# locuslab/lcp-physics

Hardware: NVIDIA H100
Metric: LCP solves/sec (LCPFunction fwd+bwd, batch=4096 x 64 contacts, fp32) (higher is better)
Workload: dtype f32 I/O and iterates; the condensed n x n KKT matrix is formed, factored and solved in f64

## Files before the change

lcp_physics_b200/csrc/lcp_condensed.cuh:

```cuda
#pragma once
#include "lcp_device.cuh"

namespace lcpb200 {
namespace cnd {

constexpr int NT = 256;
constexpr int UC = 8;
constexpr int CSMAX = 6;
constexpr int KS = 8;
constexpr int LMAX = 16;
constexpr int LU_BW = 2;
constexpr int MISC_BAND_LU = 4;
constexpr int CFLAG_DENSE_LU = 4;
constexpr int STATUS_UNSUPPORTED = -100;

struct CPlan {
  int ok;
  int n, m, e, N, NP, NS;
  int pcap;
  int wcap;
  int smem_bytes;
  int ctas_per_sm;
  int flags;
  int sbytes;
  int o_K, o_W, o_scr, o_bx, o_rdiag, o_Fd, o_Gd, o_As, o_x, o_rx, o_dx, o_qd, o_y, o_ry, o_dy,
      o_s, o_z, o_d, o_rz, o_ds, o_dz, o_rs2, o_red, o_rows, o_posof, o_clist, o_ccols, o_ncols, o_clcnt, o_misc;
};

__host__ __device__ inline size_t al16(size_t x) { return (x + 15) & ~(size_t)15; }
__host__ __device__ inline size_t scratch_bytes(int n, int m, int tsize) {
  return al16((size_t)2 * KS * m * 2) + al16((size_t)2 * KS * m * tsize) + al16((size_t)5 * m * 4) +
         al16((size_t)CSMAX * m * 2) + al16((size_t)8 * m * 4) + al16((size_t)LMAX * n * 2) + al16((size_t)n * 4) + 64;
}

inline size_t carve_plan(CPlan& P, int tsize) {
  size_t o = 0;
  const int n = P.n, m = P.m, e = P.e, NP = P.NP, pcap = P.pcap, wcap = P.wcap;
#define CND_TAKE(field, bytes) do { P.field = (int)o; o += al16((size_t)(bytes)); } while (0)
  size_t kb = (size_t)NP * NP * 8;
  if (scratch_bytes(n, m, tsize) > kb) kb = scratch_bytes(n, m, tsize);
  if ((size_t)8 * NP * 8 > kb) kb = (size_t)8 * NP * 8;
  { const size_t qn = (NP + 31) / 32, sl = (size_t)(NP / qn) * qn * qn * 32 * 8; if (sl > kb) kb = sl; }
  CND_TAKE(o_K, kb);
  CND_TAKE(o_W, (size_t)wcap * 8);
  CND_TAKE(o_scr, (size_t)pcap * 8);
  CND_TAKE(o_bx, (size_t)NP * 8);
  CND_TAKE(o_rdiag, (size_t)NP * 8);
  CND_TAKE(o_Fd, (size_t)wcap * tsize);
  CND_TAKE(o_Gd, (size_t)UC * pcap * tsize);
  CND_TAKE(o_As, (size_t)e * n * tsize);
  CND_TAKE(o_x, n * tsize); CND_TAKE(o_rx, n * tsize); CND_TAKE(o_dx, n * tsize); CND_TAKE(o_qd, n * tsize);
  CND_TAKE(o_y, e * tsize); CND_TAKE(o_ry, e * tsize); CND_TAKE(o_dy, e * tsize);
  CND_TAKE(o_s, m * tsize); CND_TAKE(o_z, m * tsize); CND_TAKE(o_d, m * tsize); CND_TAKE(o_rz, m * tsize);
  CND_TAKE(o_ds, m * tsize); CND_TAKE(o_dz, m * tsize); CND_TAKE(o_rs2, m * tsize);
  CND_TAKE(o_red, 192 * tsize);
  CND_TAKE(o_rows, pcap * 2);
  CND_TAKE(o_posof, m * 2);
  CND_TAKE(o_clist, LMAX * n * 2);
  CND_TAKE(o_ccols, UC * pcap);
  CND_TAKE(o_ncols, pcap);
  CND_TAKE(o_clcnt, n);
  CND_TAKE(o_misc, 16 * 4);
#undef CND_TAKE
  P.sbytes = 16 + (P.o_x - P.o_Fd) + (P.o_y - P.o_qd) + (P.o_misc - P.o_rows);
  return o;
}

extern __shared__ __align__(16) unsigned char cnd_smem[];

template <typename T>
struct CSmem {
  const CPlan& P;
  __device__ __forceinline__ explicit CSmem(const CPlan& p) : P(p) {}
#define CND_ACC(name, type) __device__ __forceinline__ type* name() const { return reinterpret_cast<type*>(cnd_smem + P.o_##name); }
  CND_ACC(K, double) CND_ACC(W, double) CND_ACC(scr, double) CND_ACC(bx, double) CND_ACC(rdiag, double)
  CND_ACC(Fd, T) CND_ACC(Gd, T) CND_ACC(As, T)
  CND_ACC(x, T) CND_ACC(rx, T) CND_ACC(dx, T) CND_ACC(qd, T) CND_ACC(y, T) CND_ACC(ry, T) CND_ACC(dy, T)
  CND_ACC(s, T) CND_ACC(z, T) CND_ACC(d, T) CND_ACC(rz, T) CND_ACC(ds, T) CND_ACC(dz, T) CND_ACC(rs2, T)
  CND_ACC(red, T)
  CND_ACC(rows, unsigned short) CND_ACC(posof, unsigned short) CND_ACC(clist, unsigned short)
  CND_ACC(ccols, unsigned char) CND_ACC(ncols, unsigned char) CND_ACC(clcnt, unsigned char)
  CND_ACC(misc, int)
#undef CND_ACC
};

struct Struct {
  int ncomp, cs;
  int sh;
  int m;
};

enum { CPH_STRUCT = 0, CPH_WINV, CPH_ASSEMBLE, CPH_LU, CPH_SOLVE_RHS, CPH_SOLVE_TRI, CPH_SOLVE_POST, CPH_RESID,
       CPH_STEP, CPH_GRADS, CPH_COUNT };
template <bool ON>
struct Prof {
  long long* p;
  long long t;
  __device__ __forceinline__ explicit Prof(long long* p_) : p(p_), t(0) {}
  __device__ __forceinline__ void start() { if (threadIdx.x == 0) t = clock64(); }
  __device__ __forceinline__ void lap(int ph) {
    if (threadIdx.x == 0) {
      const long long n = clock64();
      atomicAdd(reinterpret_cast<unsigned long long*>(p + ph), (unsigned long long)(n - t));
      t = n;
    }
  }
};
template <>
struct Prof<false> {
  __device__ __forceinline__ explicit Prof(long long*) {}
  __device__ __forceinline__ void start() {}
  __device__ __forceinline__ void lap(int) {}
};

template <typename T>
__device__ __forceinline__ int scan_rows(const T* __restrict__ A, int rows, int cols, T* vals, unsigned short* idx,
                                         int* cnt) {
  constexpr int CH = 8, RP = (sizeof(T) == 8) ? 2 : 4;
  const int lane = threadIdx.x & 31, warp = threadIdx.x >> 5, nw = NT >> 5;
  int bad = 0;
  if (cols <= 32 * CH) {
    for (int r0 = warp * RP; r0 < rows; r0 += nw * RP) {
      T v[RP][CH];
#pragma unroll
      for (int rr = 0; rr < RP; ++rr) {
        const T* row = A + (size_t)min(r0 + rr, rows - 1) * cols;
#pragma unroll
        for (int q = 0; q < CH; ++q) { const int j = q * 32 + lane; v[rr][q] = j < cols ? row[j] : T(0); }
      }
#pragma unroll
      for (int rr = 0; rr < RP; ++rr) {
        const int r = r0 + rr;
        if (r >= rows) break;
        int c = 0;
#pragma unroll
        for (int q = 0; q < CH; ++q) {
          const bool nz = v[rr][q] != T(0);
          const unsigned mask = __ballot_sync(FULL, nz);
          const int pos = c + __popc(mask & ((1u << lane) - 1u));
          if (nz && pos < KS) { vals[pos * rows + r] = v[rr][q]; idx[pos * rows + r] = (unsigned short)(q * 32 + lane); }
          c += __popc(mask);
        }
        if (c > KS) bad = 1;
        if (lane == 0) cnt[r] = c;
      }
    }
    return bad;
  }
  for (int r = warp; r < rows; r += nw) {
    const T* row = A + (size_t)r * cols;
    int c = 0;
    for (int j0 = 0; j0 < cols; j0 += 32 * CH) {
      T v[CH];
#pragma unroll
      for (int q = 0; q < CH; ++q) { const int j = j0 + q * 32 + lane; v[q] = j < cols ? row[j] : T(0); }
#pragma unroll
      for (int q = 0; q < CH; ++q) {
        const bool nz = v[q] != T(0);
        const unsigned mask = __ballot_sync(FULL, nz);
        const int pos = c + __popc(mask & ((1u << lane) - 1u));
        if (nz && pos < KS) { vals[pos * rows + r] = v[q]; idx[pos * rows + r] = (unsigned short)(j0 + q * 32 + lane); }
        c += __popc(mask);
      }
    }
    if (c > KS) bad = 1;
    if (lane == 0) cnt[r] = c;
  }
  return bad;
}

__device__ __forceinline__ void prefetch_l2(const void* p, size_t bytes) {
  const char* c = reinterpret_cast<const char*>(p);
  for (size_t o = (size_t)threadIdx.x * 128; o < bytes; o += (size_t)NT * 128)
    asm volatile("prefetch.global.L2 [%0];" ::"l"(c + o));
}

template <typename T>
__device__ __noinline__ bool build_structure(const CPlan& P, CSmem<T>& S, Struct& st, const T* __restrict__ Q,
                                             const T* __restrict__ G, const T* __restrict__ A,
                                             const T* __restrict__ F, int* singular) {
  const int n = P.n, m = P.m, e = P.e, tid = threadIdx.x, lane = tid & 31, warp = tid >> 5, pcap = P.pcap;
  prefetch_l2(F, (size_t)m * m * sizeof(T));
  prefetch_l2(G, (size_t)m * n * sizeof(T));
  prefetch_l2(Q, (size_t)n * n * sizeof(T));
  char* sb = reinterpret_cast<char*>(S.K());
  unsigned short* Fi = reinterpret_cast<unsigned short*>(sb);
  unsigned short* Gi = Fi + (size_t)KS * m;
  size_t o = al16((size_t)2 * KS * m * 2);
  T* Fv = reinterpret_cast<T*>(sb + o);
  T* Gv = Fv + (size_t)KS * m;
  o += al16((size_t)2 * KS * m * sizeof(T));
  int* Fcnt = reinterpret_cast<int*>(sb + o);
  int* Gcnt = Fcnt + m;
  int* label = Gcnt + m;
  int* cidx = label + m;
  int* memcnt = cidx + m;
  o += al16((size_t)5 * m * 4);
  unsigned short* memb = reinterpret_cast<unsigned short*>(sb + o);
  o += al16((size_t)CSMAX * m * 2);
  unsigned* cmap = reinterpret_cast<unsigned*>(sb + o);
  o += al16((size_t)8 * m * 4);
  unsigned short* cl_tmp = reinterpret_cast<unsigned short*>(sb + o);
  o += al16((size_t)LMAX * n * 2);
  int* cl_cnt = reinterpret_cast<int*>(sb + o);
  int* flags = S.misc();

  if (tid < 16) flags[tid] = 0;
  int bad = 0;
  for (int t = tid; t < n * n; t += NT) {
    const int i = t / n, j = t - i * n;
    const T q = Q[t];
    if (i == j) {
      S.qd()[i] = q;
      if (!(q != T(0) && isfinite((double)q))) bad |= 2;
    } else if (q != T(0)) bad |= 1;
  }
  bad |= scan_rows<T>(F, m, m, Fv, Fi, Fcnt) ? 1 : 0;
  bad |= scan_rows<T>(G, m, n, Gv, Gi, Gcnt) ? 1 : 0;
  for (int t = tid; t < e * n; t += NT) S.As()[t] = A[t];
  for (int i = tid; i < m; i += NT) { label[i] = i; memcnt[i] = 0; }
  for (int a = tid; a < n; a += NT) cl_cnt[a] = 0;
  const int anybad = __syncthreads_or(bad);
  if (anybad & 2) { *singular = 1; return false; }
  if (anybad & 1) return false;

  for (int pass = 0; pass < 64; ++pass) {
    int changed = 0;
    for (int i = tid; i < m; i += NT) {
      const int c = Fcnt[i];
      int li = ((volatile int*)label)[i];
      for (int k = 0; k < c; ++k) {
        const int j = Fi[k * m + i];
        const int lj = ((volatile int*)label)[j];
        if (lj < li) { li = lj; changed = 1; }
        else if (li < lj) { atomicMin(&label[j], li); changed = 1; }
      }
      atomicMin(&label[i], li);
    }
    if (!__syncthreads_or(changed)) break;
    if (pass == 63) return false;
  }
  if (m > 4 * NT) return false;
  int running = 0;
  for (int base = 0; base < m; base += NT) {
    const int i = base + tid;
    const bool root = i < m && label[i] == i;
    const unsigned mask = __ballot_sync(FULL, root);
    if (lane == 0) flags[8 + warp] = __popc(mask);
    __syncthreads();
    int before = running;
    for (int w = 0; w < warp; ++w) before += flags[8 + w];
    int total = 0;
    for (int w = 0; w < (NT >> 5); ++w) total += flags[8 + w];
    if (root) cidx[i] = before + __popc(mask & ((1u << lane) - 1u));
    if (i < m) {
      const int l = label[i];
      const int slot = atomicAdd(&memcnt[l], 1);
      if (slot < CSMAX) memb[l * CSMAX + slot] = (unsigned short)i;
    }
    running += total;
    __syncthreads();
  }
  const int ncomp = running;
  {
    int mx = 0;
    for (int i = tid; i < m; i += NT) mx = max(mx, memcnt[i]);
    if (mx > 0) atomicMax(&flags[3], mx);
  }
  __syncthreads();
  const int cs = flags[3];
  if (cs > CSMAX || ncomp * cs > pcap || ncomp * cs * cs > P.wcap || ncomp > 8191) return false;
  st.ncomp = ncomp; st.cs = cs; st.m = m;
  st.sh = 0;
  while ((1 << st.sh) < ncomp) ++st.sh;
  const int npos = ncomp * cs;
  for (int p = tid; p < npos; p += NT) { S.rows()[p] = 0xFFFF; S.ncols()[p] = 0; }
  for (int t = tid; t < ncomp * cs * cs; t += NT) S.Fd()[t] = T(0);
  for (int t = tid; t < UC * pcap; t += NT) { S.Gd()[t] = T(0); S.ccols()[t] = 0; }
  for (int t = tid; t < 8 * ncomp; t += NT) cmap[t] = 0u;
  __syncthreads();
  for (int i = tid; i < m; i += NT) {
    const int l = label[i], c = cidx[l], cnt = memcnt[l];
    int r = 0;
    for (int t = 0; t < cnt; ++t) r += (memb[l * CSMAX + t] < i);
    const int pos = r * ncomp + c;
    S.rows()[pos] = (unsigned short)i;
    S.posof()[i] = (unsigned short)pos;
    const int gc = Gcnt[i];
    for (int k = 0; k < gc; ++k) { const int col = Gi[k * m + i]; atomicOr(&cmap[c * 8 + (col >> 5)], 1u << (col & 31)); }
  }
  __syncthreads();
  int bad2 = 0;
  for (int i = tid; i < m; i += NT) {
    const int pos = S.posof()[i], r = pos / ncomp, c = pos - r * ncomp;
    const int fc = Fcnt[i];
    for (int k = 0; k < fc; ++k) {
      const int pj = S.posof()[Fi[k * m + i]];
      S.Fd()[(size_t)(r * cs + pj / ncomp) * ncomp + c] = Fv[k * m + i];
    }
    const int gc = Gcnt[i];
    for (int k = 0; k < gc; ++k) {
      const int col = Gi[k * m + i], wd = col >> 5;
      int p = __popc(cmap[c * 8 + wd] & ((1u << (col & 31)) - 1u));
      for (int w = 0; w < wd; ++w) p += __popc(cmap[c * 8 + w]);
      if (p < UC) { S.Gd()[(size_t)p * pcap + pos] = Gv[k * m + i]; S.ccols()[p * pcap + c] = (unsigned char)col; }
    }
  }
  for (int c = tid; c < ncomp; c += NT) {
    int cnt = 0;
#pragma unroll
    for (int w = 0; w < 8; ++w) cnt += __popc(cmap[c * 8 + w]);
    if (cnt > UC) bad2 = 1;
    S.ncols()[c] = (unsigned char)min(cnt, UC);
  }
  if (__syncthreads_or(bad2)) return false;
  int bad3 = 0;
  for (int t = tid; t < ncomp * UC; t += NT) {
    const int c = t / UC, p = t - c * UC;
    if (p < S.ncols()[c]) {
      const int a = S.ccols()[p * pcap + c];
      const int slot = atomicAdd(&cl_cnt[a], 1);
      if (slot < LMAX) cl_tmp[slot * n + a] = (unsigned short)(c * 8 + p); else bad3 = 1;
    }
  }
  if (__syncthreads_or(bad3)) return false;
  for (int t = tid; t < n * LMAX; t += NT) {
    const int a = t % n, l = t / n, cnt = cl_cnt[a];
    if (l < cnt) {
      const int v = cl_tmp[l * n + a];
      int rank = 0;
      for (int u = 0; u < cnt; ++u) rank += (cl_tmp[u * n + a] < v);
      S.clist()[rank * n + a] = (unsigned short)v;
    }
    if (l == 0) S.clcnt()[a] = (unsigned char)cnt;
  }
  __syncthreads();
  return true;
}

template <typename T>
struct EngineSoA {
  const T *mass, *inertia, *v, *fext;
  const T *normal, *p1, *p2;
  const T *mu, *rest;
  const int32_t *b1, *b2;
  const int32_t* nc_s;
  int nb, nc;
  int mode;
  T dt;
  T *p_s, *h_s;
};

template <typename T>
__device__ __forceinline__ void contact_row(T p1x, T p1y, T p2x, T p2y, T dx, T dy, T (&r1)[3], T (&r2)[3]) {
  r1[0] = p1x * dy - p1y * dx; r1[1] = dx; r1[2] = dy;
  r2[0] = -(p2x * dy - p2y * dx); r2[1] = -dx; r2[2] = -dy;
}

template <typename T>
__device__ __noinline__ bool build_structure_soa(const CPlan& P, CSmem<T>& S, Struct& st, const EngineSoA<T>& e_,
                                                 int sc, const T* __restrict__ A, int* singular) {
  const int n = P.n, e = P.e, tid = threadIdx.x, pcap = P.pcap;
  const int nb = e_.nb, ncs = e_.nc, cs = e_.mode == 0 ? 4 : 1;
  const int nc = e_.nc_s ? e_.nc_s[sc] : e_.nc;
  const int m = cs * nc;
  const int32_t* tb1 = e_.b1 + (e_.nc_s ? (size_t)sc * ncs : 0);
  const int32_t* tb2 = e_.b2 + (e_.nc_s ? (size_t)sc * ncs : 0);
  char* sb = reinterpret_cast<char*>(S.K());
  unsigned short* cl_tmp = reinterpret_cast<unsigned short*>(sb);
  int* cl_cnt = reinterpret_cast<int*>(sb + al16((size_t)LMAX * n * 2));
  if (n != 3 * nb || nc < 0 || nc > ncs || m > P.m || nc * cs > pcap || nc * cs * cs > P.wcap) return false;
// ... 699 lines not shown
template <typename T>
__device__ __noinline__ void fwd_store_best(const CFwdArgs<T>& a, CSmem<T> S, int m, int sc) {
  const CPlan& P = a.P;
  const int n = P.n, e = P.e, tid = threadIdx.x;
  for (int i = tid; i < n; i += NT) a.zhat[(size_t)sc * n + i] = S.x()[i];
  for (int i = tid; i < m; i += NT) { a.lam[(size_t)sc * P.m + i] = S.z()[i]; a.slack[(size_t)sc * P.m + i] = S.s()[i]; }
  for (int i = tid; i < e; i += NT) a.nu[(size_t)sc * e + i] = S.y()[i];
}

template <typename T>
__device__ __noinline__ void fwd_centering(CSmem<T> S, int m, T mu, T sz) {
  const int tid = threadIdx.x;
  T stz, sts;
  get_steps(S.z(), S.dz(), S.s(), S.ds(), m, S.red(), stz, sts);
  const T alpha_aff = nan_min(nan_min(stz, sts), T(1));
  T t3[1] = {0};
  for (int i = tid; i < m; i += NT) t3[0] += (S.s()[i] + alpha_aff * S.ds()[i]) * (S.z()[i] + alpha_aff * S.dz()[i]);
  block_reduce<T, 1>(t3, OpSum(), T(0), S.red());
  const T ratio = t3[0] / sz;
  const T sig = ratio * ratio * ratio;
  const T musig = -mu * sig;
  for (int i = tid; i < m; i += NT) S.rs2()[i] = (musig + S.ds()[i] * S.dz()[i]) / S.s()[i];
  __syncthreads();
}

template <typename T>
__device__ __noinline__ void fwd_step(const CPlan& P, CSmem<T> S, int m) {
  const int n = P.n, e = P.e, tid = threadIdx.x;
  for (int i = tid; i < n; i += NT) S.dx()[i] += S.rx()[i];
  for (int i = tid; i < m; i += NT) { S.ds()[i] += S.rz()[i]; S.dz()[i] += S.rs2()[i]; }
  for (int i = tid; i < e; i += NT) S.dy()[i] += S.ry()[i];
  __syncthreads();
  T stz, sts;
  get_steps(S.z(), S.dz(), S.s(), S.ds(), m, S.red(), stz, sts);
  const T alpha = nan_min(T(0.999) * nan_min(stz, sts), T(1));
  for (int i = tid; i < n; i += NT) S.x()[i] += alpha * S.dx()[i];
  for (int i = tid; i < m; i += NT) { S.s()[i] += alpha * S.ds()[i]; S.z()[i] += alpha * S.dz()[i]; }
  for (int i = tid; i < e; i += NT) S.y()[i] += alpha * S.dy()[i];
  __syncthreads();
}

template <typename T, int NS, int CS, typename PF>
__device__ __forceinline__ void forward_scene(const CFwdArgs<T>& a, CSmem<T>& S, const Struct& st, PF& pf, int sc) {
  const CPlan& P = a.P;
  const int m = st.m;
  {
    const int n = P.n, e = P.e, tid = threadIdx.x;
    const T* h = a.h + (size_t)sc * P.m;
    const T* b = e > 0 ? a.b + (size_t)sc * e : nullptr;
    for (int i = tid; i < m; i += NT) { S.d()[i] = T(1); S.rs2()[i] = T(0); S.rz()[i] = -h[i]; }
    for (int i = tid; i < n; i += NT) S.rx()[i] = a.p[(size_t)sc * n + i];
    for (int i = tid; i < e; i += NT) S.ry()[i] = -b[i];
    __syncthreads();
  }
  factor_kkt<T, NS, CS>(P, S, st, pf);
  solve_kkt<T, CS, NS>(P, S, st, pf, S.rx(), S.rs2(), S.rz(), P.e > 0 ? S.ry() : nullptr, S.x(), S.s(), S.z(), S.y());
  if (m == 0) {
    fwd_store_best<T>(a, S, 0, sc);
    if (threadIdx.x == 0) { a.status[sc] = 2; a.iters[sc] = 0; if (a.resid) a.resid[sc] = T(0); }
    return;
  }
  {
    const int tid = threadIdx.x;
    T mn[2] = {INFINITY, INFINITY};
    for (int i = tid; i < m; i += NT) { mn[0] = nan_min(mn[0], S.s()[i]); mn[1] = nan_min(mn[1], S.z()[i]); }
    block_reduce<T, 2>(mn, OpMin(), (T)INFINITY, S.red());
    for (int i = tid; i < m; i += NT) {
      if (mn[0] <= T(0)) S.s()[i] -= mn[0] - T(1);
      if (mn[1] <= T(0)) S.z()[i] -= mn[1] - T(1);
    }
    __syncthreads();
  }

  T best = nan("");
  bool have_best = false;
  int not_improved = 0, status = 0, it = 0;
  for (it = 0; it < a.max_iter; ++it) {
    const SzResid<T> r = fwd_residuals<T, CS>(a, S, st, sc);
    pf.lap(CPH_RESID);
    const T mu = fabs(r.sz / T(m));

    bool improved;
    if (!have_best) { improved = true; have_best = true; not_improved = 0; }
    else { improved = r.resid < best; not_improved = improved ? 0 : not_improved + 1; }
    if (improved) {
      best = r.resid;
      fwd_store_best<T>(a, S, m, sc);
    }
    if (not_improved == a.not_improved_lim) { status = 1; ++it; break; }
    if (best < a.eps) { status = 2; ++it; break; }
    if (mu > T(1e100)) { status = 3; ++it; break; }

    for (int i = threadIdx.x; i < m; i += NT) S.d()[i] = S.z()[i] / S.s()[i];
    __syncthreads();
    factor_kkt<T, NS, CS>(P, S, st, pf);

    solve_kkt<T, CS, NS>(P, S, st, pf, S.rx(), S.z(), S.rz(), P.e > 0 ? S.ry() : nullptr, S.dx(), S.ds(), S.dz(), S.dy());
    fwd_centering<T>(S, m, mu, r.sz);
    pf.lap(CPH_STEP);
    solve_kkt<T, CS, NS>(P, S, st, pf, nullptr, S.rs2(), nullptr, nullptr, S.rx(), S.rz(), S.rs2(), S.ry());
    fwd_step<T>(P, S, m);
    pf.lap(CPH_STEP);
  }
  if (threadIdx.x == 0) { a.status[sc] = status; a.iters[sc] = it; if (a.resid) a.resid[sc] = best; }
}

template <typename T, int NS, bool PROF>
__global__ void __launch_bounds__(NT, (NS <= 6) ? 2 : 1) cond_forward_kernel(const __grid_constant__ CFwdArgs<T> a) {
  const CPlan& P = a.P;
  CSmem<T> S(P);
  const int n = P.n, m = P.m, e = P.e, tid = threadIdx.x;
  __shared__ int singular_s;
  const T NANV = nan("");
  Prof<PROF> pf(PROF ? a.prof + (size_t)blockIdx.x * CPH_COUNT : nullptr);
  for (int sc = blockIdx.x; sc < a.B; sc += gridDim.x) {
    if (tid == 0) singular_s = 0;
    __syncthreads();
    pf.start();
    Struct st;
    const bool ok = a.soa.mass
        ? build_structure_soa<T>(P, S, st, a.soa, sc, e > 0 ? a.A + (size_t)sc * e * n : nullptr, &singular_s)
        : build_structure<T>(P, S, st, a.Q + (size_t)sc * n * n, a.G + (size_t)sc * m * n,
                             e > 0 ? a.A + (size_t)sc * e * n : nullptr, a.F + (size_t)sc * m * m, &singular_s);
    __syncthreads();
    if (a.ssave) save_structure(P, st, ok, a.ssave + (size_t)sc * P.sbytes);
    pf.lap(CPH_STRUCT);
    if (!ok) {
      if (singular_s) {
        for (int i = tid; i < n; i += NT) a.zhat[(size_t)sc * n + i] = NANV;
        for (int i = tid; i < m; i += NT) { a.lam[(size_t)sc * m + i] = NANV; a.slack[(size_t)sc * m + i] = NANV; }
        for (int i = tid; i < e; i += NT) a.nu[(size_t)sc * e + i] = NANV;
        if (tid == 0) { a.status[sc] = -1; a.iters[sc] = 0; if (a.resid) a.resid[sc] = NANV; }
      } else if (tid == 0) {
        a.status[sc] = STATUS_UNSUPPORTED;
        a.iters[sc] = 0;
      }
      __syncthreads();
      continue;
    }
    if constexpr (LU_BW < NS - 1) mark_band_lu<T>(P, S, st);
    switch (st.cs) {
      case 1: forward_scene<T, NS, 1>(a, S, st, pf, sc); break;
      case 2: forward_scene<T, NS, 2>(a, S, st, pf, sc); break;
      case 3: forward_scene<T, NS, 3>(a, S, st, pf, sc); break;
      case 4: forward_scene<T, NS, 4>(a, S, st, pf, sc); break;
      case 5: forward_scene<T, NS, 5>(a, S, st, pf, sc); break;
      default: forward_scene<T, NS, 6>(a, S, st, pf, sc); break;
    }
    __syncthreads();
  }
}

template <typename T, typename F>
__device__ __forceinline__ void write_outer(T* __restrict__ o, int rows, int cols, F f) {
  constexpr int V = 16 / (int)sizeof(T);
  const int tid = threadIdx.x;
  if (cols % V == 0 && (reinterpret_cast<size_t>(o) & 15) == 0) {
    const int cv = cols / V, total = rows * cv;
    const int di = NT / cv, dj = NT - di * cv;
    int i = tid / cv, jv = tid - i * cv;
    for (int t = tid; t < total; t += NT) {
      const int j = jv * V;
      if (V == 4) {
        float4 w;
        w.x = (float)f(i, j); w.y = (float)f(i, j + 1); w.z = (float)f(i, j + 2); w.w = (float)f(i, j + 3);
        reinterpret_cast<float4*>(o)[t] = w;
      } else {
        double2 w;
        w.x = (double)f(i, j); w.y = (double)f(i, j + 1);
        reinterpret_cast<double2*>(o)[t] = w;
      }
      i += di; jv += dj;
      if (jv >= cv) { jv -= cv; ++i; }
    }
  } else {
    int i = tid / cols, j = tid - i * cols;
    const int di = NT / cols, dj = NT - di * cols;
    for (size_t t = tid; t < (size_t)rows * cols; t += NT) {
      o[t] = f(i, j);
      i += di; j += dj;
      if (j >= cols) { j -= cols; ++i; }
    }
  }
}

template <typename T, int CS, typename PF>
__device__ __forceinline__ void backward_grads(const CBwdArgs<T>& a, CSmem<T>& S, const Struct& st, PF& pf, int sc, int so) {
  const CPlan& P = a.P;
  const int n = P.n, m = st.m, e = P.e, tid = threadIdx.x;
  const T* dx = S.dx(); const T* dlam = S.dz(); const T* dnu = S.dy();
  if (a.soa.mass) {
    const EngineSoA<T>& E = a.soa;
    const int nc = st.ncomp, nb = E.nb, ncs = E.nc;
    const int32_t* tb1 = E.b1 + (E.nc_s ? (size_t)sc * ncs : 0);
    const int32_t* tb2 = E.b2 + (E.nc_s ? (size_t)sc * ncs : 0);
    const T* v = E.v + (size_t)sc * n;
    const T* zh_ = S.x(); const T* lm = S.z();
    for (int c = tid; c < ncs; c += NT) {
      const size_t ic = (size_t)sc * ncs + c, oc = (size_t)so * ncs + c;
      if (c >= nc) {
        if (a.dnormal) { a.dnormal[oc * 2] = 0; a.dnormal[oc * 2 + 1] = 0; }
        if (a.dp1) { a.dp1[oc * 2] = 0; a.dp1[oc * 2 + 1] = 0; }
        if (a.dp2) { a.dp2[oc * 2] = 0; a.dp2[oc * 2 + 1] = 0; }
        if (a.drest) a.drest[oc] = 0;
        if (a.dmu) a.dmu[oc] = 0;
        continue;
      }
      const T nx = E.normal[ic * 2], ny = E.normal[ic * 2 + 1];
      const T p1x = E.p1[ic * 2], p1y = E.p1[ic * 2 + 1], p2x = E.p2[ic * 2], p2y = E.p2[ic * 2 + 1];
      const bool two = tb2[c] < nb;
      const int j1 = 3 * tb1[c], j2 = two ? 3 * tb2[c] : j1;
      const T rc = E.rest[ic];
      const T dhc = -dlam[c] * (E.mode == 0 ? T(1) : T(1));
      T gnx = 0, gny = 0, g1x = 0, g1y = 0, g2x = 0, g2y = 0, jcv = 0;
      const int nrows = E.mode == 0 ? 3 : 1;
      const int rows_[3] = {c, nc + 2 * c, nc + 2 * c + 1};
      const T dxs[3] = {nx, ny, -ny}, dys[3] = {ny, -nx, nx};
      for (int q = 0; q < nrows; ++q) {
        const T ddx_ = dxs[q], ddy_ = dys[q];
        const int i = rows_[q];
        T g[6];
        for (int t = 0; t < 3; ++t) {
          g[t] = dlam[i] * zh_[j1 + t] + lm[i] * dx[j1 + t];
          g[3 + t] = two ? dlam[i] * zh_[j2 + t] + lm[i] * dx[j2 + t] : T(0);
        }
        if (q == 0) {
          const T row[6] = {p1x * ddy_ - p1y * ddx_, ddx_, ddy_, -(p2x * ddy_ - p2y * ddx_), -ddx_, -ddy_};
          for (int t = 0; t < 3; ++t) jcv += row[t] * v[j1 + t] + row[3 + t] * (two ? v[j2 + t] : T(0));
          const T hs_ = E.mode == 0 ? rc : (T(1) - rc);
          for (int t = 0; t < 3; ++t) { g[t] += dhc * hs_ * v[j1 + t]; g[3 + t] += dhc * hs_ * (two ? v[j2 + t] : T(0)); }
        }
        const T gdx = -p1y * g[0] + g[1] + p2y * g[3] - g[4];
        const T gdy = p1x * g[0] + g[2] - p2x * g[3] - g[5];
        g1x += ddy_ * g[0]; g1y += -ddx_ * g[0];
        g2x += -ddy_ * g[3]; g2y += ddx_ * g[3];
        if (q == 0) { gnx += gdx; gny += gdy; }
        else if (q == 1) { gny += gdx; gnx += -gdy; }
        else { gny += -gdx; gnx += gdy; }
      }
      if (a.dnormal) { a.dnormal[oc * 2] = gnx; a.dnormal[oc * 2 + 1] = gny; }
      if (a.dp1) { a.dp1[oc * 2] = g1x; a.dp1[oc * 2 + 1] = g1y; }
      if (a.dp2) { a.dp2[oc * 2] = g2x; a.dp2[oc * 2 + 1] = g2y; }
      if (a.drest) a.drest[oc] = E.mode == 0 ? dhc * jcv : -dhc * jcv;
      if (a.dmu) a.dmu[oc] = E.mode == 0 ? -(dlam[3 * nc + c] * lm[c]) : T(0);
    }
    for (int j = tid; j < n; j += NT) {
      const int body = j / 3, comp = j - 3 * body;
      const T md = comp == 0 ? E.inertia[(size_t)sc * nb + body] : E.mass[(size_t)sc * nb + body];
      const T dpj = E.mode == 0 ? dx[j] : T(0);
      if (a.dfext) a.dfext[(size_t)so * n + j] = E.dt * dpj;
      if (a.dv) {
        T acc = md * dpj;
        const int cnt = S.clcnt()[j];
        for (int l = 0; l < cnt; ++l) {
          const int cp = S.clist()[l * n + j], c = cp >> 3, pslot = cp & 7;
          const T hs_ = E.mode == 0 ? E.rest[(size_t)sc * ncs + c] : (T(1) - E.rest[(size_t)sc * ncs + c]);
          acc += -dlam[c] * hs_ * S.Gd()[(size_t)pslot * P.pcap + c];
        }
        a.dv[(size_t)so * n + j] = acc;
      }
      const T dqjj = dx[j] * zh_[j];
      if (comp == 0 && a.dinertia) a.dinertia[(size_t)so * nb + body] = dqjj + dpj * v[j];
    }
    __syncthreads();
    for (int body = tid; body < nb; body += NT) {
      if (!a.dmass) break;
      T acc = 0;
      for (int comp = 1; comp < 3; ++comp) {
        const int j = 3 * body + comp;
        acc += dx[j] * zh_[j] + (E.mode == 0 ? dx[j] : T(0)) * v[j];
      }
      a.dmass[(size_t)so * nb + body] = acc;
    }
    if (a.db && e > 0) for (int i = tid; i < e; i += NT) a.db[(size_t)so * e + i] = -dnu[i];
    if (a.dA && e > 0) {
      T* o = a.dA + (size_t)so * e * n;
      for (int i = 0; i < e; ++i)
        for (int j = tid; j < n; j += NT) o[(size_t)i * n + j] = dnu[i] * S.x()[j] + S.y()[i] * dx[j];
    }
    if (tid == 0 && a.done) a.done[sc] = 1;
    __syncthreads();
    pf.lap(CPH_GRADS);
    return;
  }
  if (a.dp) for (int i = tid; i < n; i += NT) a.dp[(size_t)so * n + i] = dx[i];
  if (a.dh) for (int i = tid; i < m; i += NT) a.dh[(size_t)so * m + i] = -dlam[i];
  if (a.db && e > 0) for (int i = tid; i < e; i += NT) a.db[(size_t)so * e + i] = -dnu[i];
  if (a.dG)
    write_outer<T>(a.dG + (size_t)so * m * n, m, n, [&](int i, int j) { return dlam[i] * S.x()[j] + S.z()[i] * dx[j]; });
  if (a.dF)
    write_outer<T>(a.dF + (size_t)so * m * m, m, m, [&](int i, int j) { return -(dlam[i] * S.z()[j]); });
  if (a.dA && e > 0)
    write_outer<T>(a.dA + (size_t)so * e * n, e, n, [&](int i, int j) { return dnu[i] * S.x()[j] + S.y()[i] * dx[j]; });
  if (a.dQ)
    write_outer<T>(a.dQ + (size_t)so * n * n, n, n, [&](int i, int j) { return T(0.5) * (dx[i] * S.x()[j] + S.x()[i] * dx[j]); });
  if (tid == 0 && a.done) a.done[sc] = 1;
  __syncthreads();
  pf.lap(CPH_GRADS);
}

template <typename T, int NS, int CS, typename PF>
__device__ __forceinline__ void backward_scene(const CBwdArgs<T>& a, CSmem<T>& S, const Struct& st, PF& pf, int sc,
                                               int r0, int r1) {
  const CPlan& P = a.P;
  const int n = P.n, m = st.m, e = P.e, tid = threadIdx.x;
  const T* zh = a.zhat + (size_t)sc * n;
  const T* lam = a.lam + (size_t)sc * P.m;
  const T* slk = a.slack + (size_t)sc * P.m;
  const T* nu = e > 0 ? a.nu + (size_t)sc * e : nullptr;
  for (int i = tid; i < n; i += NT) S.x()[i] = zh[i];
  for (int i = tid; i < m; i += NT) {
    T d = lam[i] / slk[i];
    if (sizeof(T) == 8) d = d > T(1e10) ? T(1e10) : (d < T(1e-10) ? T(1e-10) : d);
    S.z()[i] = lam[i]; S.s()[i] = slk[i]; S.d()[i] = d;
  }
  for (int i = tid; i < e; i += NT) S.y()[i] = nu[i];
  __syncthreads();
  const bool exact = (a.flags & 1u) != 0;
  factor_kkt<T, NS, CS>(P, S, st, pf, exact);
  for (int r = r0; r < r1; ++r) {
    const int so = r * a.B + sc;
    for (int i = tid; i < n; i += NT) S.rx()[i] = a.g[(size_t)so * n + i];
    for (int i = tid; i < m; i += NT) S.rs2()[i] = T(0);
    __syncthreads();
    solve_kkt<T, CS, NS>(P, S, st, pf, S.rx(), S.rs2(), nullptr, nullptr, S.dx(), S.ds(), S.dz(), S.dy(), exact);
    backward_grads<T, CS>(a, S, st, pf, sc, so);
  }
}

template <typename T, int NS, bool PROF>
__global__ void __launch_bounds__(NT, (NS <= 6) ? 2 : 1) cond_backward_kernel(const __grid_constant__ CBwdArgs<T> a) {
  const CPlan& P = a.P;
  CSmem<T> S(P);
  const int n = P.n, m = P.m, e = P.e, tid = threadIdx.x;
  __shared__ int singular_s;
  Prof<PROF> pf(PROF ? a.prof + (size_t)blockIdx.x * CPH_COUNT : nullptr);
  for (int w = blockIdx.x; w < a.B * a.chunks; w += gridDim.x) {
    const int sc = w / a.chunks, k = w - sc * a.chunks;
    if (a.only && !a.only[sc]) continue;
    if (tid == 0) singular_s = 0;
    __syncthreads();
    pf.start();
    Struct st;
    const bool ok = a.soa.mass
        ? build_structure_soa<T>(P, S, st, a.soa, sc, e > 0 ? a.A + (size_t)sc * e * n : nullptr, &singular_s)
        : a.sload
              ? load_structure(P, st, a.sload + (size_t)sc * P.sbytes)
              : build_structure<T>(P, S, st, a.Q + (size_t)sc * n * n, a.G + (size_t)sc * m * n,
                                   e > 0 ? a.A + (size_t)sc * e * n : nullptr, a.F + (size_t)sc * m * m, &singular_s);
    __syncthreads();
    pf.lap(CPH_STRUCT);
    if (!ok) {
      if (tid == 0 && a.done) a.done[sc] = 0;
      __syncthreads();
      continue;
    }
    if constexpr (LU_BW < NS - 1) mark_band_lu<T>(P, S, st);
    const int r0 = (int)((long long)a.R * k / a.chunks), r1 = (int)((long long)a.R * (k + 1) / a.chunks);
    switch (st.cs) {
      case 1: backward_scene<T, NS, 1>(a, S, st, pf, sc, r0, r1); break;
      case 2: backward_scene<T, NS, 2>(a, S, st, pf, sc, r0, r1); break;
      case 3: backward_scene<T, NS, 3>(a, S, st, pf, sc, r0, r1); break;
      case 4: backward_scene<T, NS, 4>(a, S, st, pf, sc, r0, r1); break;
      case 5: backward_scene<T, NS, 5>(a, S, st, pf, sc, r0, r1); break;
      default: backward_scene<T, NS, 6>(a, S, st, pf, sc, r0, r1); break;
    }
    __syncthreads();
  }
}


template <typename T>
struct EngineTangents {
  const T *mass, *inertia, *v, *fext, *normal, *p1, *p2, *mu, *rest, *A, *b;
};

template <typename T>
struct CJvpArgs {
  CPlan P;
  int B, R, chunks;
  const T *Q, *G, *A, *F;
  const T *zhat, *nu, *lam, *slack;
  EngineSoA<T> soa;
  EngineTangents<T> t;
  const T *tQ, *tp, *tG, *th, *tF;
  int* done;
  const int* only;
  const unsigned char* sload;
  T* dz;
  long long* prof;
};

template <typename T>
__device__ __forceinline__ void contact_row_tangent(T p1x, T p1y, T p2x, T p2y, T dx, T dy, T t1x, T t1y, T t2x,
                                                    T t2y, T tdx, T tdy, T (&r1)[3], T (&r2)[3]) {
  r1[0] = t1x * dy + p1x * tdy - t1y * dx - p1y * tdx; r1[1] = tdx; r1[2] = tdy;
  r2[0] = -(t2x * dy + p2x * tdy - t2y * dx - p2y * tdx); r2[1] = -tdx; r2[2] = -tdy;
}

template <typename T, typename L>
__device__ __forceinline__ void engine_jvp_rhs(const EngineSoA<T>& E, const EngineTangents<T>& t, L lay, int sc, int so,
                                            int n, int e, int nc) {
  const int tid = threadIdx.x, nb = E.nb, ncs = E.nc;
  const int32_t* tb1 = E.b1 + (E.nc_s ? (size_t)sc * ncs : 0);
  const int32_t* tb2 = E.b2 + (E.nc_s ? (size_t)sc * ncs : 0);
  const T* v = E.v + (size_t)sc * n;
  const T* tv = t.v ? t.v + (size_t)so * n : nullptr;
  const T* zh = lay.x(); const T* lm = lay.z();
  T* rz = lay.rz();
  auto tget = [](const T* p, size_t i) { return p ? p[i] : T(0); };
  for (int k = tid; k < nc; k += NT) {
    const size_t ic = (size_t)sc * ncs + k, oc = (size_t)so * ncs + k;
    const int b1 = tb1[k], b2 = tb2[k];
    const bool two = b2 < nb;
    const T nx = E.normal[ic * 2], ny = E.normal[ic * 2 + 1];
    const T p1x = E.p1[ic * 2], p1y = E.p1[ic * 2 + 1], p2x = E.p2[ic * 2], p2y = E.p2[ic * 2 + 1];
    const T tnx = tget(t.normal, oc * 2), tny = tget(t.normal, oc * 2 + 1);
    const T t1x = tget(t.p1, oc * 2), t1y = tget(t.p1, oc * 2 + 1);
    const T t2x = tget(t.p2, oc * 2), t2y = tget(t.p2, oc * 2 + 1);
    T r1[3], r2[3], d1[3], d2[3];
    contact_row<T>(p1x, p1y, p2x, p2y, nx, ny, r1, r2);
    contact_row_tangent<T>(p1x, p1y, p2x, p2y, nx, ny, t1x, t1y, t2x, t2y, tnx, tny, d1, d2);
    T jv = 0, tjv = 0, gz = 0;
#pragma unroll
    for (int q = 0; q < 3; ++q) {
      const int j1 = 3 * b1 + q;
      jv += r1[q] * v[j1];
      tjv += d1[q] * v[j1] + (tv ? r1[q] * tv[j1] : T(0));
      gz += d1[q] * zh[j1];
      if (two) {
        const int j2 = 3 * b2 + q;
        jv += r2[q] * v[j2];
        tjv += d2[q] * v[j2] + (tv ? r2[q] * tv[j2] : T(0));
        gz += d2[q] * zh[j2];
      }
    }
    const T rc = E.rest[ic], trc = tget(t.rest, oc);
    if (E.mode == 0) {
      rz[lay.row(0, k)] = gz - (trc * jv + rc * tjv);
      contact_row_tangent<T>(p1x, p1y, p2x, p2y, ny, -nx, t1x, t1y, t2x, t2y, tny, -tnx, d1, d2);
      T fz = 0;
#pragma unroll
      for (int q = 0; q < 3; ++q) { fz += d1[q] * zh[3 * b1 + q]; if (two) fz += d2[q] * zh[3 * b2 + q]; }
      rz[lay.row(1, k)] = fz;
      rz[lay.row(2, k)] = -fz;
      rz[lay.row(3, k)] = -(tget(t.mu, oc) * lm[k]);
    } else {
      rz[lay.row(0, k)] = gz - (tjv * (T(1) - rc) - trc * jv);
// ... 184 lines not shown
```

Baseline: 305,500.

## Vectorize input scans with evict-first loads and streaming outer-product gradient stores

Replaces the L2 prefetch and scalar scans of Q, F and G with 16-byte non-allocating loads that carry an L2 evict-first policy. The F and G sparsity scan is now batched over several rows per warp, with ballot-based position counting. The outer-product gradient writer is restructured so each thread keeps its column vectors in registers and writes rows using streaming (__stcs) stores. The intent is to cut global-memory instruction count and cache pollution in the bandwidth-heavy structure build and gradient phases. It adds a scalar-IO flag fallback and more register pressure from the unrolled row batches.

Result: faster. 312,000 (median of 6 runs) (+2.1%).

```diff
diff --git a/lcp_physics_b200/csrc/lcp_condensed.cuh b/lcp_physics_b200/csrc/lcp_condensed.cuh
--- a/lcp_physics_b200/csrc/lcp_condensed.cuh
+++ b/lcp_physics_b200/csrc/lcp_condensed.cuh
@@ -12,6 +12,7 @@
 constexpr int LU_BW = 2;
 constexpr int MISC_BAND_LU = 4;
 constexpr int CFLAG_DENSE_LU = 4;
+constexpr int CFLAG_SCALAR_IO = 8;
 constexpr int STATUS_UNSUPPORTED = -100;
 
 struct CPlan {
@@ -175,14 +176,96 @@
     asm volatile("prefetch.global.L2 [%0];" ::"l"(c + o));
 }
 
+__device__ __forceinline__ unsigned long long l2_evict_first() {
+  unsigned long long pol;
+  asm("createpolicy.fractional.L2::evict_first.b64 %0, 1.0;" : "=l"(pol));
+  return pol;
+}
+__device__ __forceinline__ void ld16_once(const float* p, float (&v)[4], unsigned long long pol) {
+  asm("ld.global.nc.L1::no_allocate.L2::cache_hint.v4.f32 {%0, %1, %2, %3}, [%4], %5;"
+      : "=f"(v[0]), "=f"(v[1]), "=f"(v[2]), "=f"(v[3]) : "l"(p), "l"(pol));
+}
+__device__ __forceinline__ void ld16_once(const double* p, double (&v)[2], unsigned long long pol) {
+  asm("ld.global.nc.L1::no_allocate.L2::cache_hint.v2.f64 {%0, %1}, [%2], %3;"
+      : "=d"(v[0]), "=d"(v[1]) : "l"(p), "l"(pol));
+}
+
+template <typename T, int RP, int NQ>
+__device__ __forceinline__ int scan_rows_v16(const T* __restrict__ A, int rows, int cols, T* vals, unsigned short* idx,
+                                             int* cnt) {
+  constexpr int V = 16 / (int)sizeof(T), CW = 32 * V, NB = V == 4 ? 3 : 2;
+  const int lane = threadIdx.x & 31, warp = threadIdx.x >> 5, nw = NT >> 5;
+  const unsigned below = (1u << lane) - 1u;
+  const unsigned long long pol = l2_evict_first();
+  int bad = 0;
+  for (int r0 = warp * RP; r0 < rows; r0 += nw * RP) {
+    T v[RP][NQ][V];
+#pragma unroll
+    for (int rr = 0; rr < RP; ++rr) {
+      const T* row = A + (size_t)min(r0 + rr, rows - 1) * cols;
+#pragma unroll
+      for (int q = 0; q < NQ; ++q) {
+        const int j = q * CW + lane * V;
+        if (j < cols) ld16_once(row + j, v[rr][q], pol);
+        else {
+#pragma unroll
+          for (int u = 0; u < V; ++u) v[rr][q][u] = T(0);
+        }
+      }
+    }
+#pragma unroll
+    for (int rr = 0; rr < RP; ++rr) {
+      const int r = r0 + rr;
+      if (r >= rows) break;
+      int c = 0;
+#pragma unroll
+      for (int q = 0; q < NQ; ++q) {
+        int k = 0;
+#pragma unroll
+        for (int u = 0; u < V; ++u) k += v[rr][q][u] != T(0);
+        int pos = c, tot = 0;
+#pragma unroll
+        for (int b = 0; b < NB; ++b) {
+          const unsigned mb = __ballot_sync(FULL, (k >> b) & 1);
+          pos += __popc(mb & below) << b;
+          tot += __popc(mb) << b;
+        }
+#pragma unroll
+        for (int u = 0; u < V; ++u) {
+          if (v[rr][q][u] != T(0)) {
+            if (pos < KS) { vals[pos * rows + r] = v[rr][q][u]; idx[pos * rows + r] = (unsigned short)(q * CW + lane * V + u); }
+            ++pos;
+          }
+        }
+        c += tot;
+      }
+      if (c > KS) bad = 1;
+      if (lane == 0) cnt[r] = c;
+    }
+  }
+  return bad;
+}
+
+constexpr int SCAN_LD16 = 8;
+template <typename T>
+__device__ __forceinline__ int scan_rows_fast(const T* __restrict__ A, int rows, int cols, T* vals, unsigned short* idx,
+                                              int* cnt, bool scalar) {
+  constexpr int V = 16 / (int)sizeof(T), CW = 32 * V;
+  if (!scalar && cols % V == 0 && (reinterpret_cast<size_t>(A) & 15) == 0) {
+    if (cols <= CW) return scan_rows_v16<T, SCAN_LD16, 1>(A, rows, cols, vals, idx, cnt);
+    if (cols <= 2 * CW) return scan_rows_v16<T, SCAN_LD16 / 2, 2>(A, rows, cols, vals, idx, cnt);
+    if (cols <= 4 * CW) return scan_rows_v16<T, SCAN_LD16 / 4, 4>(A, rows, cols, vals, idx, cnt);
+  }
+  prefetch_l2(A, (size_t)rows * cols * sizeof(T));
+  return scan_rows<T>(A, rows, cols, vals, idx, cnt);
+}
+
 template <typename T>
 __device__ __noinline__ bool build_structure(const CPlan& P, CSmem<T>& S, Struct& st, const T* __restrict__ Q,
                                              const T* __restrict__ G, const T* __restrict__ A,
                                              const T* __restrict__ F, int* singular) {
   const int n = P.n, m = P.m, e = P.e, tid = threadIdx.x, lane = tid & 31, warp = tid >> 5, pcap = P.pcap;
-  prefetch_l2(F, (size_t)m * m * sizeof(T));
-  prefetch_l2(G, (size_t)m * n * sizeof(T));
-  prefetch_l2(Q, (size_t)n * n * sizeof(T));
+  const bool scalar = (P.flags & CFLAG_SCALAR_IO) != 0;
   char* sb = reinterpret_cast<char*>(S.K());
   unsigned short* Fi = reinterpret_cast<unsigned short*>(sb);
   unsigned short* Gi = Fi + (size_t)KS * m;
@@ -207,16 +290,37 @@
 
   if (tid < 16) flags[tid] = 0;
   int bad = 0;
-  for (int t = tid; t < n * n; t += NT) {
-    const int i = t / n, j = t - i * n;
-    const T q = Q[t];
-    if (i == j) {
-      S.qd()[i] = q;
-      if (!(q != T(0) && isfinite((double)q))) bad |= 2;
-    } else if (q != T(0)) bad |= 1;
-  }
-  bad |= scan_rows<T>(F, m, m, Fv, Fi, Fcnt) ? 1 : 0;
-  bad |= scan_rows<T>(G, m, n, Gv, Gi, Gcnt) ? 1 : 0;
+  constexpr int V = 16 / (int)sizeof(T);
+  if (!scalar && n % V == 0 && (reinterpret_cast<size_t>(Q) & 15) == 0) {
+    const unsigned long long pol = l2_evict_first();
+    const int cv = n / V, di = NT / cv, dj = NT - di * cv;
+    int i = tid / cv, jv = tid - i * cv;
+#pragma unroll 3
+    for (int t = tid; t < n * cv; t += NT) {
+      T q[V];
+      ld16_once(Q + (size_t)t * V, q, pol);
+#pragma unroll
+      for (int u = 0; u < V; ++u) {
+        if (jv * V + u == i) {
+          S.qd()[i] = q[u];
+          if (!(q[u] != T(0) && isfinite((double)q[u]))) bad |= 2;
+        } else if (q[u] != T(0)) bad |= 1;
+      }
+      i += di; jv += dj;
+      if (jv >= cv) { jv -= cv; ++i; }
+    }
+  } else {
+    for (int t = tid; t < n * n; t += NT) {
+      const int i = t / n, j = t - i * n;
+      const T q = Q[t];
+      if (i == j) {
+        S.qd()[i] = q;
+        if (!(q != T(0) && isfinite((double)q))) bad |= 2;
+      } else if (q != T(0)) bad |= 1;
+    }
+  }
+  bad |= scan_rows_fast<T>(F, m, m, Fv, Fi, Fcnt, scalar) ? 1 : 0;
+  bad |= scan_rows_fast<T>(G, m, n, Gv, Gi, Gcnt, scalar) ? 1 : 0;
   for (int t = tid; t < e * n; t += NT) S.As()[t] = A[t];
   for (int i = tid; i < m; i += NT) { label[i] = i; memcnt[i] = 0; }
   for (int a = tid; a < n; a += NT) cl_cnt[a] = 0;
@@ -1222,32 +1326,31 @@
 }
 
 template <typename T, typename F>
-__device__ __forceinline__ void write_outer(T* __restrict__ o, int rows, int cols, F f) {
+__device__ __forceinline__ void write_outer(T* __restrict__ o, int rows, int cols, const T* ra, const T* rb,
+                                            const T* ca, const T* cb, bool scalar, F f) {
   constexpr int V = 16 / (int)sizeof(T);
+  using VT = typename std::conditional<V == 4, float4, double2>::type;
   const int tid = threadIdx.x;
-  if (cols % V == 0 && (reinterpret_cast<size_t>(o) & 15) == 0) {
-    const int cv = cols / V, total = rows * cv;
-    const int di = NT / cv, dj = NT - di * cv;
-    int i = tid / cv, jv = tid - i * cv;
-    for (int t = tid; t < total; t += NT) {
-      const int j = jv * V;
-      if (V == 4) {
-        float4 w;
-        w.x = (float)f(i, j); w.y = (float)f(i, j + 1); w.z = (float)f(i, j + 2); w.w = (float)f(i, j + 3);
-        reinterpret_cast<float4*>(o)[t] = w;
-      } else {
-        double2 w;
-        w.x = (double)f(i, j); w.y = (double)f(i, j + 1);
-        reinterpret_cast<double2*>(o)[t] = w;
-      }
-      i += di; jv += dj;
-      if (jv >= cv) { jv -= cv; ++i; }
+  if (!scalar && cols % V == 0 && (reinterpret_cast<size_t>(o) & 15) == 0) {
+    const int cv = cols / V, R = cv <= NT ? NT / cv : 1, i0 = tid / cv, jv0 = tid - i0 * cv;
+    if (i0 >= R) return;
+    for (int jv = jv0; jv < cv; jv += NT) {
+      union { VT v; T e[V]; } a, b, w;
+      a.v = reinterpret_cast<const VT*>(ca)[jv];
+      b.v = reinterpret_cast<const VT*>(cb)[jv];
+      VT* out = reinterpret_cast<VT*>(o) + jv;
+      for (int i = i0; i < rows; i += R) {
+        const T ri = ra[i], si = rb[i];
+#pragma unroll
+        for (int u = 0; u < V; ++u) w.e[u] = f(ri, si, a.e[u], b.e[u]);
+        __stcs(out + (size_t)i * cv, w.v);
+      }
     }
   } else {
     int i = tid / cols, j = tid - i * cols;
     const int di = NT / cols, dj = NT - di * cols;
     for (size_t t = tid; t < (size_t)rows * cols; t += NT) {
-      o[t] = f(i, j);
+      o[t] = f(ra[i], rb[i], ca[j], cb[j]);
       i += di; j += dj;
       if (j >= cols) { j -= cols; ++i; }
     }
@@ -1356,14 +1459,19 @@
   if (a.dp) for (int i = tid; i < n; i += NT) a.dp[(size_t)so * n + i] = dx[i];
   if (a.dh) for (int i = tid; i < m; i += NT) a.dh[(size_t)so * m + i] = -dlam[i];
   if (a.db && e > 0) for (int i = tid; i < e; i += NT) a.db[(size_t)so * e + i] = -dnu[i];
+  const bool scalar = (P.flags & CFLAG_SCALAR_IO) != 0;
   if (a.dG)
-    write_outer<T>(a.dG + (size_t)so * m * n, m, n, [&](int i, int j) { return dlam[i] * S.x()[j] + S.z()[i] * dx[j]; });
+    write_outer<T>(a.dG + (size_t)so * m * n, m, n, dlam, S.z(), S.x(), dx, scalar,
+                   [](T dl, T lm, T xj, T dxj) { return dl * xj + lm * dxj; });
   if (a.dF)
-    write_outer<T>(a.dF + (size_t)so * m * m, m, m, [&](int i, int j) { return -(dlam[i] * S.z()[j]); });
+    write_outer<T>(a.dF + (size_t)so * m * m, m, m, dlam, dlam, S.z(), S.z(), scalar,
+                   [](T dl, T, T lj, T) { return -(dl * lj); });
   if (a.dA && e > 0)
-    write_outer<T>(a.dA + (size_t)so * e * n, e, n, [&](int i, int j) { return dnu[i] * S.x()[j] + S.y()[i] * dx[j]; });
+    write_outer<T>(a.dA + (size_t)so * e * n, e, n, dnu, S.y(), S.x(), dx, scalar,
+                   [](T dn, T yi, T xj, T dxj) { return dn * xj + yi * dxj; });
   if (a.dQ)
-    write_outer<T>(a.dQ + (size_t)so * n * n, n, n, [&](int i, int j) { return T(0.5) * (dx[i] * S.x()[j] + S.x()[i] * dx[j]); });
+    write_outer<T>(a.dQ + (size_t)so * n * n, n, n, dx, S.x(), S.x(), dx, scalar,
+                   [](T dxi, T xi, T xj, T dxj) { return T(0.5) * (dxi * xj + xi * dxj); });
   if (tid == 0 && a.done) a.done[sc] = 1;
   __syncthreads();
   pf.lap(CPH_GRADS);
```
